# karfly/learnable-triangulation-pytorch

Hardware: NVIDIA H100
Metric: volumetric samples/sec (4-view 384x384, 64^3 grid) (higher is better)
Workload: dtype fp16x3 (split-fp16 operands, 3 wgmma products per term, fp32 accumulate)

## Files before the change

### include/lt_b200.h

```cpp
#ifndef LT_B200_H
#define LT_B200_H

#include <stddef.h>
#include <stdint.h>

#ifdef __cplusplus
extern "C" {
#endif

enum lt_status {
  LT_OK = 0,
  LT_ERR_INVALID = -1,
  LT_ERR_CUDA = -2,
  LT_ERR_UNSUPPORTED = -3
};

enum lt_format { LT_FMT_F32 = 0, LT_FMT_S32 = 1 };

enum lt_agg { LT_AGG_SUM = 0, LT_AGG_MAX = 1, LT_AGG_SOFTMAX = 2, LT_AGG_CONF = 3 };

enum lt_conv_impl {
  LT_CONV_SIMT = 0,
  LT_CONV_TC = 1,
  LT_CONV_TC1 = 2,
  LT_CONV_TC_FOLD = 3,
};

enum lt_residual { LT_RES_NONE = 0, LT_RES_BEFORE_RELU = 1, LT_RES_AFTER_RELU = 2 };

typedef struct lt_options {
  int tc_persist;
  int tc_splitk;
  int tc_bres;
  int tc_direct_epilogue;
  int fold_fast_issue;
  int fold_debug;
  int softargmax_stream;
  int unproject_v2;
  int unproject_cpl;
  int unproject_lb;
  int unproject_brick;
  int unproject_brick_order;
  int pair_nt, pair_stages;
  int pair_prof;
  int pair_direct_out;
  int pair_two_acc;
  int fold_pair;
  int fold_direct;
  int fold_fullw;
} lt_options;
void lt_default_options(lt_options* o);
int lt_get_options(lt_options* o);
int lt_set_options(const lt_options* o);

int lt_version(void);
const char* lt_last_error_string(void);

int lt_device_info(int* sm_count, int* cc_major, int* cc_minor);

int lt_coord_volume_fwd(const float* position, const float* center, const float* step, const float* rot,
                        float* out, int B, int n, int transfer_cmu, void* stream);

int lt_unproject_aggregate_fwd(const float* features, const float* proj, const float* coord, const float* conf,
                               void* out, int out_format, int B, int V, int C, int h, int w, long nvox,
                               int agg, void* stream);

int lt_unproject_partial_fwd(const float* features, const float* proj, const float* coord, const float* conf,
                             float* partial, int B, int V_local, int C, int h, int w, long nvox,
                             int agg, void* stream);
int lt_unproject_finalize_fwd(const float* partial, void* out, int out_format, int B, int C, long nvox,
                              int agg, void* stream);

int lt_unproject_push_fwd(const float* features, const float* proj, const float* coord, const float* conf,
                          float* const* peer_buffers , int n_peers, int src_rank,
                          int B, int V_local, int C, int h, int w, long nvox, int agg, void* stream);
int lt_unproject_reduce_finalize_fwd(const float* slots, int nslots, void* out, int out_format, int B, int C, long nvox,
                                     int agg, void* stream);

int lt_feature_scatter_fwd(const float* feats, float* const* peer_buffers, int n_peers, int view_rank, int B, int V_local,
                           int V, long row_elems, void* stream);

int lt_unproject_aggregate_bwd(const float* features, const float* proj, const float* coord, const float* conf,
// ... 17 lines not shown
int lt_softargmax3d_finish_fwd(const float* logits, long batch_stride, long voxel_stride, const float* coord, float* volumes_out,
                               float* keypoints_out, void* workspace, size_t workspace_bytes, int B, int J, long nvox, int G,
                               float multiplier, int softmax, void* stream);

typedef struct lt_conv_desc {
  int N, ID, IH, IW, Cin;
  int OD, OH, OW, Cout;
  int KD, KH, KW;
  int sd, sh, sw;
  int pd, ph, pw;
  int FD, FH, FW, FC;
  int osd, osh, osw;
  int ood, ooh, oow;
  int relu;
  int residual;
  int in_format, out_format;
  int ogd, ogh, ogw;
  int reserved0;
  void* workspace;
  size_t workspace_bytes;
} lt_conv_desc;

int lt_conv_nd_fwd(const lt_conv_desc* desc, const void* in, const void* weight, const float* scale,
                   const float* shift, const void* residual, void* out, int impl, void* stream);

size_t lt_conv_tc_weight_bytes(int taps, int Cin, int Cout);

typedef struct lt_conv_tc_launch_plan {
  int nt;
  int m_tiles, n_tiles;
  int chunks;
  int splits;
  int grid;
} lt_conv_tc_launch_plan;
int lt_conv_tc_plan(const lt_conv_desc* desc, int sm_count, int splitk, lt_conv_tc_launch_plan* plan);
int lt_conv_tc_pack_weights(const float* w_tap_ci_co, void* packed, int taps, int Cin, int Cout, void* stream);

int lt_absmax_fwd(const float* w, long n, unsigned int* out_bits, void* stream);
int lt_conv_gather_weights_fwd(const float* w, long base, long s_td, long s_th, long s_tw, long s_ci, long s_co, int KD, int KH, int KW,
                               int Cin, int CinP, int Cout, int CoutP, const unsigned int* absmax_bits, float* out, int out_ld,
                               int out_col0, void* stream);
int lt_fold_bn_fwd(const float* gamma, const float* beta, const float* mean, const float* var, const float* conv_bias, float eps,
                   int C, int CP, const unsigned int* absmax_bits, int accum_steps, float* scale, float* shift, void* stream);

int lt_v2v_tail_fwd(const void* x, const void* w1, const void* w2, const void* w3, const float* scale1, const float* shift1,
                    const float* scale2, const float* shift2, const float* scale3, const float* bias3, float* logits, long rows, int FC,
                    void* stream);
int lt_v2v_tail_stats_fwd(const void* x, const void* w1, const void* w2, const void* w3, const float* scale1, const float* shift1,
                          const float* scale2, const float* shift2, const float* scale3, const float* bias3, float* logits, int B,
                          long nvox, int FC, const float* coord, int J, float multiplier, int softmax, void* workspace,
                          size_t workspace_bytes, int* n_partials, void* stream);

size_t lt_conv_wgrad_workspace_bytes(const lt_conv_desc* desc);
typedef struct lt_conv_wgrad_launch_plan {
  int nwg;
  int ngroups;
  int m_tiles;
  int splits;
  int stages;
} lt_conv_wgrad_launch_plan;
int lt_conv_wgrad_plan(const lt_conv_desc* desc, int sm_count, lt_conv_wgrad_launch_plan* plan);
int lt_conv_wgrad_fwd(const lt_conv_desc* desc, const void* in, const void* grad_out, const unsigned int* grad_absmax_bits, int Cin,
                      int Cout, float* grad_w, void* workspace, size_t workspace_bytes, void* stream);

size_t lt_conv_fold_weight_bytes(int K, int Cout);
int lt_conv_fold_pack_weights(const float* w_tap_ci_co, void* packed, int K, int Cout, void* stream);
// ... 69 lines not shown
```

### learnable-triangulation-pytorch_b200/capi.py

```python
import ctypes
import os

import torch

from . import build as _build

_HERE = os.path.dirname(os.path.abspath(__file__))
LIB_PATH = os.path.join(_HERE, "liblt_b200.so")

FMT_F32, FMT_S32 = 0, 1
AGG = {"sum": 0, "max": 1, "softmax": 2, "conf": 3, "conf_norm": 3}
CONV_SIMT, CONV_TC, CONV_TC1, CONV_TC_FOLD = 0, 1, 2, 3
RES_NONE, RES_BEFORE_RELU, RES_AFTER_RELU = 0, 1, 2

c_int, c_long, c_float, c_void_p, c_size_t = ctypes.c_int, ctypes.c_long, ctypes.c_float, ctypes.c_void_p, ctypes.c_size_t


class ConvDesc(ctypes.Structure):
    _fields_ = [(n, c_int) for n in (
        "N", "ID", "IH", "IW", "Cin",
        "OD", "OH", "OW", "Cout",
        "KD", "KH", "KW",
        "sd", "sh", "sw",
        "pd", "ph", "pw",
        "FD", "FH", "FW", "FC",
        "osd", "osh", "osw",
        "ood", "ooh", "oow",
        "relu", "residual", "in_format", "out_format", "ogd", "ogh", "ogw", "reserved0")] + [("workspace", c_void_p), ("workspace_bytes", c_size_t)]


class ConvTcPlan(ctypes.Structure):
    _fields_ = [(n, c_int) for n in ("nt", "m_tiles", "n_tiles", "chunks", "splits", "grid")]


class ConvWgradPlan(ctypes.Structure):
    _fields_ = [(n, c_int) for n in ("nwg", "ngroups", "m_tiles", "splits", "stages")]


class Options(ctypes.Structure):
    _fields_ = [(n, c_int) for n in ("tc_persist", "tc_splitk", "tc_bres", "tc_direct_epilogue", "fold_fast_issue", "fold_debug",
                                     "softargmax_stream", "unproject_v2", "unproject_cpl", "unproject_lb", "unproject_brick", "unproject_brick_order", "pair_nt", "pair_stages", "pair_prof", "pair_direct_out", "pair_two_acc", "fold_pair", "fold_direct", "fold_fullw")]


OPTIONS_ENV_PREFIX = "LT_OPT_"

SIGNATURES = {
    "lt_default_options": (None, [ctypes.POINTER(Options)]),
    "lt_get_options": (c_int, [ctypes.POINTER(Options)]),
    "lt_set_options": (c_int, [ctypes.POINTER(Options)]),
    "lt_version": (c_int, []),
    "lt_last_error_string": (ctypes.c_char_p, []),
    "lt_device_info": (c_int, [ctypes.POINTER(c_int)] * 3),
    "lt_coord_volume_fwd": (c_int, [c_void_p] * 5 + [c_int, c_int, c_int, c_void_p]),
    "lt_unproject_aggregate_fwd": (c_int, [c_void_p] * 5 + [c_int] * 6 + [c_long, c_int, c_void_p]),
    "lt_unproject_partial_fwd": (c_int, [c_void_p] * 5 + [c_int] * 5 + [c_long, c_int, c_void_p]),
    "lt_unproject_finalize_fwd": (c_int, [c_void_p, c_void_p, c_int, c_int, c_int, c_long, c_int, c_void_p]),
    "lt_unproject_push_fwd": (c_int, [c_void_p] * 4 + [ctypes.POINTER(c_void_p), c_int, c_int] + [c_int] * 5 + [c_long, c_int, c_void_p]),
    "lt_unproject_reduce_finalize_fwd": (c_int, [c_void_p, c_int, c_void_p, c_int, c_int, c_int, c_long, c_int, c_void_p]),
    "lt_feature_scatter_fwd": (c_int, [c_void_p, ctypes.POINTER(c_void_p), c_int, c_int, c_int, c_int, c_int, c_long, c_void_p]),
    "lt_unproject_aggregate_bwd": (c_int, [c_void_p] * 7 + [c_int] * 5 + [c_long, c_int, c_void_p]),
    "lt_softargmax3d_bwd": (c_int, [c_void_p] * 6 + [c_int, c_int, c_long, c_float, c_int, c_void_p]),
    "lt_unproject_aggregate_bwd_geom_workspace_bytes": (c_size_t, [c_int, c_int, c_long]),
    "lt_unproject_aggregate_bwd_geom": (c_int, [c_void_p] * 10 + [c_size_t] + [c_int] * 5 + [c_long, c_int, c_void_p]),
    "lt_softargmax3d_coord_bwd": (c_int, [c_void_p] * 3 + [c_int, c_int, c_long, c_int, c_void_p]),
    "lt_test_unproject_aggregate_bwd_geom_host": (c_int, [c_void_p] * 9 + [c_int] * 5 + [c_long, c_int]),
    "lt_test_softargmax3d_coord_bwd_host": (c_int, [c_void_p] * 3 + [c_int, c_int, c_long]),
    "lt_test_unproject_aggregate_bwd_host": (c_int, [c_void_p] * 7 + [c_int] * 5 + [c_long, c_int]),
    "lt_test_softargmax3d_bwd_host": (c_int, [c_void_p] * 5 + [c_int, c_int, c_long, c_float, c_int]),
    "lt_softargmax3d_workspace_bytes": (c_size_t, [c_int, c_int, c_long]),
    "lt_softargmax3d_fwd": (c_int, [c_void_p, c_long, c_long, c_long, c_void_p, c_void_p, c_void_p, c_void_p, c_size_t,
                                    c_int, c_int, c_long, c_float, c_int, c_void_p]),
    "lt_conv_nd_fwd": (c_int, [ctypes.POINTER(ConvDesc)] + [c_void_p] * 6 + [c_int, c_void_p]),
    "lt_conv_tc_weight_bytes": (c_size_t, [c_int, c_int, c_int]),
    "lt_conv_tc_plan": (c_int, [ctypes.POINTER(ConvDesc), c_int, c_int, ctypes.POINTER(ConvTcPlan)]),
# ... 447 lines not shown
```

### learnable-triangulation-pytorch_b200/csrc/capi.cu

```cuda
#include "common.cuh"
#include <string.h>

namespace lt {

char* err_buf() {
  static thread_local char buf[512] = {0};
  return buf;
}

int fail(int code, const char* fmt, ...) {
  va_list ap;
  va_start(ap, fmt);
  vsnprintf(err_buf(), 512, fmt, ap);
  va_end(ap);
  return code;
}

static lt_options make_default_options() {
  lt_options o;
  o.tc_persist = 1; o.tc_splitk = 1; o.tc_bres = 1; o.tc_direct_epilogue = 0;
  o.fold_fast_issue = 1; o.fold_debug = 0;
  o.softargmax_stream = 1;
  o.unproject_v2 = 1; o.unproject_cpl = 4; o.unproject_lb = 0;
  o.unproject_brick = 0; o.unproject_brick_order = 2;
  o.pair_nt = 0; o.pair_stages = 0;
  o.pair_prof = 0;
  o.pair_direct_out = 1;
  o.pair_two_acc = 1;
  o.fold_pair = 1;
  o.fold_direct = 0;
  o.fold_fullw = 1;
  return o;
}
static lt_options g_options = make_default_options();
const lt_options& opts() { return g_options; }

int sm_count() {
  static thread_local int cached_dev = -1, cached = 0;
  int dev = 0;
  if (cudaGetDevice(&dev) != cudaSuccess) return 132;
  if (dev != cached_dev) {
    int n = 0;
    if (cudaDeviceGetAttribute(&n, cudaDevAttrMultiProcessorCount, dev) != cudaSuccess || n <= 0) n = 132;
    cached = n;
    cached_dev = dev;
  }
  return cached;
}

int conv_simt_fwd(const lt_conv_desc* d, const void* in, const void* weight, const float* scale, const float* shift,
                  const void* residual, void* out, void* stream);
int conv_tc_fwd_terms(const lt_conv_desc* d, const void* in, const void* weight, const float* scale, const float* shift,
                      const void* residual, void* out, int terms, void* stream);

int conv_fold_fwd(const lt_conv_desc* d, const void* in, const void* weight, const float* scale, const float* shift,
                  const void* residual, void* out, void* stream);

}

extern "C" int lt_version(void) { return 203; }

extern "C" void lt_default_options(lt_options* o) {
  if (o) *o = lt::make_default_options();
}
extern "C" int lt_get_options(lt_options* o) {
  if (!o) return lt::fail(LT_ERR_INVALID, "lt_get_options: null pointer");
  *o = lt::g_options;
  return LT_OK;
}
extern "C" int lt_set_options(const lt_options* o) {
  using namespace lt;
  LT_REQUIRE(o, "lt_set_options: null pointer");
  LT_REQUIRE(o->unproject_cpl == 4 || o->unproject_cpl == 8, "lt_set_options: unproject_cpl must be 4 or 8");
  LT_REQUIRE(o->tc_persist >= 0 && o->tc_persist <= 2, "lt_set_options: tc_persist must be 0, 1 or 2");
  g_options = *o;
  return LT_OK;
}

extern "C" const char* lt_last_error_string(void) { return lt::err_buf(); }

extern "C" int lt_device_info(int* sm_count, int* cc_major, int* cc_minor) {
  int dev = 0;
  if (cudaGetDevice(&dev) != cudaSuccess) return lt::fail(LT_ERR_CUDA, "no CUDA device");
  cudaDeviceProp prop;
  if (cudaGetDeviceProperties(&prop, dev) != cudaSuccess) return lt::fail(LT_ERR_CUDA, "cudaGetDeviceProperties failed");
  if (sm_count) *sm_count = prop.multiProcessorCount;
  if (cc_major) *cc_major = prop.major;
  if (cc_minor) *cc_minor = prop.minor;
  return LT_OK;
}

extern "C" int lt_conv_nd_fwd(const lt_conv_desc* d, const void* in, const void* weight, const float* scale,
                              const float* shift, const void* residual, void* out, int impl, void* stream) {
  using namespace lt;
  LT_REQUIRE(d && in && weight && scale && shift && out, "conv_nd: null pointer");
  LT_REQUIRE(d->N > 0 && d->ID > 0 && d->IH > 0 && d->IW > 0 && d->Cin > 0, "conv_nd: bad input dims");
  LT_REQUIRE(d->OD > 0 && d->OH > 0 && d->OW > 0 && d->Cout > 0, "conv_nd: bad output dims");
  LT_REQUIRE(d->KD > 0 && d->KH > 0 && d->KW > 0 && d->sd > 0 && d->sh > 0 && d->sw > 0, "conv_nd: bad filter/stride");
  LT_REQUIRE(d->osd > 0 && d->osh > 0 && d->osw > 0, "conv_nd: bad output scale");
  const int gd = d->ogd > 1 ? d->ogd : 1, gh = d->ogh > 1 ? d->ogh : 1, gw = d->ogw > 1 ? d->ogw : 1;
  LT_REQUIRE((d->OD - 1) * d->osd + d->ood < d->FD && (d->OH - 1) * d->osh + d->ooh < d->FH && (d->OW - 1) * d->osw + d->oow < d->FW &&
                 d->ood + gd - 1 < d->FD && d->ooh + gh - 1 < d->FH && d->oow + gw - 1 < d->FW && d->ood >= 0 && d->ooh >= 0 &&
                 d->oow >= 0,
             "conv_nd: output mapping exceeds the output tensor");
  LT_REQUIRE(gd * gh * gw == 1 || impl == LT_CONV_TC || impl == LT_CONV_TC1,
             "conv_nd: grouped output (ogd/ogh/ogw) is only implemented by the tensor-core kernels");
  LT_REQUIRE(d->residual == LT_RES_NONE || residual, "conv_nd: residual requested but pointer is null");
// ... 8 lines not shown
```

### learnable-triangulation-pytorch_b200/csrc/conv_tc.cu

```cuda
#include "tc_common.cuh"
#include "conv_tc_params.cuh"
#include <stdlib.h>
#include <string.h>

namespace lt {

constexpr int kTcThreads = 384;

struct TcUnit {
  int m, n0, z, q_begin, nchunks;
};
__device__ __forceinline__ TcUnit tc_unit(const TcParams& p, int u, int m_tiles, int nchunks_all) {
  TcUnit w;
  const int n = u % p.n_tiles;
  u /= p.n_tiles;
  w.m = u % m_tiles;
  w.z = u / m_tiles;
  w.n0 = n * p.Nt;
  w.q_begin = (int)(((long)w.z * nchunks_all) / p.splits);
  w.nchunks = (int)(((long)(w.z + 1) * nchunks_all) / p.splits) - w.q_begin;
  return w;
}
__device__ __forceinline__ void tc_tile_origin(const TcParams& p, int t, int& ow0, int& oh0, int& od0, int& nb0) {
  ow0 = (t % p.tw) * p.bw; t /= p.tw;
  oh0 = (t % p.th) * p.bh; t /= p.th;
  od0 = (t % p.td) * p.bd;
  nb0 = (t / p.td) * p.bn;
}

constexpr int kSlabBytes = 128 * 128;
__host__ __device__ constexpr int tc_epi_bytes(int nt, int splits) { return (nt >= 32 && splits == 1) ? nt / 32 * kSlabBytes : 0; }

__device__ __forceinline__ void epi_slab(const TcParams& p, int co, int& g, int& c) {
  g = p.n_maps > 1 ? co / p.oc : 0;
  const int ch = co - g * p.oc;
  c = p.out_format == LT_FMT_F32 ? ch : 2 * ch;
}

__device__ __forceinline__ uint32_t sw128(int row, int b) {
  return (uint32_t)(row * 128 + ((((b >> 4) ^ row) & 7) << 4) + (b & 15));
}

template <int NT>
__global__ void __launch_bounds__(kTcThreads, 1) conv_tc_kernel(const __grid_constant__ CUtensorMap tmA,
                                                                const __grid_constant__ CUtensorMap tmB,
                                                                const __grid_constant__ TcEpiMaps tmE, const TcParams p) {
  extern __shared__ uint8_t smem_raw[];
  uint8_t* smem = reinterpret_cast<uint8_t*>((reinterpret_cast<uintptr_t>(smem_raw) + 1023) & ~(uintptr_t)1023);
  constexpr int kStage = kATileBytes + NT * 128;
  const int epi_bytes = tc_epi_bytes(NT, p.splits);
  const bool staged = epi_bytes > 0;
  uint8_t* ebuf = smem + (size_t)p.stages * kStage;
  uint64_t* full = reinterpret_cast<uint64_t*>(ebuf + epi_bytes);
  uint64_t* empty = full + p.stages;
  uint64_t* efull = empty + p.stages;
  uint64_t* edone = efull + 1;

  const int wg = __shfl_sync(0xffffffffu, (int)(threadIdx.x >> 7), 0);
  const int lane = threadIdx.x & 31;
  const int m_tiles = p.tw * p.th * p.td * p.tn;
  const int units = m_tiles * p.n_tiles * p.splits;
  const int nchunks_all = p.KD * p.KH * p.KW * p.CB;

  if (threadIdx.x == 0) {
    for (int s = 0; s < p.stages; ++s) { mbar_init(&full[s], 1); mbar_init(&empty[s], 2); }
    mbar_init(efull, 1);
    mbar_init(edone, 256);
    fence_barrier_init();
    prefetch_tmap(&tmA);
    prefetch_tmap(&tmB);
  }
  __syncthreads();

  if (wg == 0) {
    regs_release_producer();
    if (staged && threadIdx.x == 32) {
      uint32_t eph = 0;
      for (int u = blockIdx.x; u < units; u += gridDim.x) {
        const TcUnit w = tc_unit(p, u, m_tiles, nchunks_all);
        int ow0, oh0, od0, nb0;
        tc_tile_origin(p, w.m, ow0, oh0, od0, nb0);
        bulk_wait_read0();
        if (p.residual != LT_RES_NONE) {
          mbar_expect_tx(efull, (uint32_t)epi_bytes);
          for (int sl = 0; sl < NT / 32; ++sl) {
            int g, c;
            epi_slab(p, w.n0 + 32 * sl, g, c);
            tma_load_5d(ebuf + sl * kSlabBytes, &tmE.res[g], efull, c, ow0, oh0, od0, nb0);
          }
        } else {
          mbar_arrive_local(efull);
        }
        mbar_wait(edone, eph);
        eph ^= 1u;
        for (int sl = 0; sl < NT / 32; ++sl) {
          int g, c;
          epi_slab(p, w.n0 + 32 * sl, g, c);
          tma_store_5d(&tmE.out[g], ebuf + sl * kSlabBytes, c, ow0, oh0, od0, nb0);
        }
        bulk_commit();
      }
      bulk_wait0();
    }
    if (threadIdx.x < 32) {
      int s = 0;
      uint32_t ph = 0;
      for (int u = blockIdx.x; u < units; u += gridDim.x) {
        const TcUnit w = tc_unit(p, u, m_tiles, nchunks_all);
        int ow0, oh0, od0, nb0;
        tc_tile_origin(p, w.m, ow0, oh0, od0, nb0);
        int tap = w.q_begin / p.CB, cb = w.q_begin - tap * p.CB;
        int kw = tap % p.KW, kh = (tap / p.KW) % p.KH, kd = tap / (p.KW * p.KH);
        const int ax = ow0 * p.sw - p.pw, ay = oh0 * p.sh - p.ph, az = od0 * p.sd - p.pd, bn0 = w.n0 * p.b_nmul;
        for (int q = 0, qa = w.q_begin; q < w.nchunks; ++q, ++qa) {
          mbar_wait(&empty[s], ph ^ 1u);
          uint8_t* a_dst = smem + (size_t)s * kStage;
          if (elect_one()) {
            mbar_expect_tx(&full[s], (uint32_t)kStage);
            tma_load_5d(a_dst, &tmA, &full[s], cb * 64, ax + kw, ay + kh, az + kd, nb0);
            tma_load_2d(a_dst + kATileBytes, &tmB, &full[s], qa * p.b_step0, qa * p.b_step1 + bn0);
          }
          __syncwarp();
          if (++cb == p.CB) { cb = 0; if (++kw == p.KW) { kw = 0; if (++kh == p.KH) { kh = 0; ++kd; } } }
          if (++s == p.stages) { s = 0; ph ^= 1u; }
        }
      }
    }
    return;
  }

  regs_claim_consumer();
  const int g = wg - 1;
  float d1[NT / 2], d2[NT / 2];
#pragma unroll
  for (int i = 0; i < NT / 2; ++i) { d1[i] = 0.f; d2[i] = 0.f; }
  const int r0 = g * 64 + ((threadIdx.x >> 5) & 3) * 16 + (lane >> 2);
  const int c2 = 2 * (lane & 3);
  const uint32_t ring0 = smem_u32(smem);
  int s = 0;
  uint32_t ph = 0, eph = 0;
  for (int u = blockIdx.x; u < units; u += gridDim.x) {
    const TcUnit w = tc_unit(p, u, m_tiles, nchunks_all);
    int prev = -1;
    for (int q = 0; q < w.nchunks; ++q) {
      mbar_wait(&full[s], ph);
      const uint32_t a_addr = ring0 + (uint32_t)(s * kStage) + (uint32_t)(g * 64 * 128);
      const uint32_t b_addr = ring0 + (uint32_t)(s * kStage) + kATileBytes;
      const uint64_t ad = make_sw128_desc(a_addr), bd = make_sw128_desc(b_addr);
      const uint32_t acc = (q == 0) ? 0u : 1u;
      wg_fence();
      if (p.terms == 3) {
        wgmma_f16<NT>(d1, ad, bd, acc);
        wgmma_f16<NT>(d1, ad + 2, bd + 2, 1u);
        wgmma_f16<NT>(d2, ad, bd + 4, acc);
        wgmma_f16<NT>(d2, ad + 2, bd + 6, 1u);
        wgmma_f16<NT>(d2, ad + 4, bd, 1u);
        wgmma_f16<NT>(d2, ad + 6, bd + 2, 1u);
      } else if (p.terms == 1) {
        wgmma_f16<NT>(d1, ad, bd, acc);
        wgmma_f16<NT>(d1, ad + 2, bd + 2, 1u);
      } else {
        wgmma_f16<NT>(d1, ad, bd, acc);
        wgmma_f16<NT>(d1, ad + 2, bd + 2, 1u);
        wgmma_f16<NT>(d1, ad + 4, bd + 4, 1u);
        wgmma_f16<NT>(d1, ad + 6, bd + 6, 1u);
      }
      wg_commit();
      wg_wait<1>();
      if (prev >= 0 && (threadIdx.x & 127) == 0) mbar_arrive_local(&empty[prev]);
      prev = s;
      if (++s == p.stages) { s = 0; ph ^= 1u; }
    }
    wg_wait<0>();
    if (prev >= 0 && (threadIdx.x & 127) == 0) mbar_arrive_local(&empty[prev]);
    wg_fence_regs(d1);
    wg_fence_regs(d2);

    if (p.splits > 1) {
#pragma unroll
      for (int h = 0; h < 2; ++h) {
        float* wrow = p.ws + (((size_t)w.z * m_tiles + w.m) * 128 + r0 + 8 * h) * p.ws_ld + w.n0;
#pragma unroll
        for (int i = 0; i < NT / 8; ++i) {
          const int k = 4 * i + 2 * h;
          const float v0 = (p.terms == 3) ? fmaf(d2[k], kLoInv, d1[k]) : d1[k];
          const float v1 = (p.terms == 3) ? fmaf(d2[k + 1], kLoInv, d1[k + 1]) : d1[k + 1];
          *reinterpret_cast<float2*>(wrow + 8 * i + c2) = make_float2(v0, v1);
        }
      }
      continue;
    }
    if constexpr (NT >= 32) {
      mbar_wait(efull, eph);
      eph ^= 1u;
      const uint32_t e0 = smem_u32(ebuf);
      auto fc_ok = [&](int co) {
        int ch;
        long pix;
        epilogue_target(p, co, 0, ch, pix);
        return ch < p.FC;
      };
      float2 sc = make_float2(0.f, 0.f), sh = sc;
      if (fc_ok(w.n0 + c2)) {
        sc = __ldg(reinterpret_cast<const float2*>(p.scale + w.n0 + c2));
        sh = __ldg(reinterpret_cast<const float2*>(p.shift + w.n0 + c2));
      }
#pragma unroll
      for (int i = 0; i < NT / 8; ++i) {
        const int co = w.n0 + 8 * i + c2;
        const bool ok = fc_ok(co);
        float2 sc_next = sc, sh_next = sh;
        if (i + 1 < NT / 8 && fc_ok(co + 8)) {
          sc_next = __ldg(reinterpret_cast<const float2*>(p.scale + co + 8));
          sh_next = __ldg(reinterpret_cast<const float2*>(p.shift + co + 8));
        }
        const uint32_t slab = e0 + (uint32_t)((i >> 2) * kSlabBytes);
        const int cc = 8 * (i & 3) + c2;
#pragma unroll
        for (int h = 0; h < 2 && ok; ++h) {
          const int row = r0 + 8 * h;
          const int k = 4 * i + 2 * h;
          float v0 = (p.terms == 3) ? fmaf(d2[k], kLoInv, d1[k]) : d1[k];
          float v1 = (p.terms == 3) ? fmaf(d2[k + 1], kLoInv, d1[k + 1]) : d1[k + 1];
          v0 = fmaf(v0, sc.x, sh.x);
          v1 = fmaf(v1, sc.y, sh.y);
          if (p.out_format == LT_FMT_F32) {
            const uint32_t a = slab + sw128(row, 4 * cc);
            float2 r = make_float2(0.f, 0.f);
            if (p.residual != LT_RES_NONE) r = lds_f2(a);
            if (p.residual == LT_RES_BEFORE_RELU) { v0 += r.x; v1 += r.y; }
            if (p.relu) { v0 = fmaxf(v0, 0.f); v1 = fmaxf(v1, 0.f); }
            if (p.residual == LT_RES_AFTER_RELU) { v0 += r.x; v1 += r.y; }
            sts_f2(a, make_float2(v0, v1));
          } else {
            const uint32_t ahi = slab + sw128(row, 2 * cc), alo = slab + sw128(row, 64 + 2 * cc);
            float2 r = make_float2(0.f, 0.f);
            if (p.residual != LT_RES_NONE) {
              const uint32_t rh = lds32(ahi), rl = lds32(alo);
              const float2 a = __half22float2(*reinterpret_cast<const __half2*>(&rh));
              const float2 b = __half22float2(*reinterpret_cast<const __half2*>(&rl));
              r = make_float2(fmaf(b.x, kLoInv, a.x), fmaf(b.y, kLoInv, a.y));
            }
            if (p.residual == LT_RES_BEFORE_RELU) { v0 += r.x; v1 += r.y; }
            if (p.relu) { v0 = fmaxf(v0, 0.f); v1 = fmaxf(v1, 0.f); }
            if (p.residual == LT_RES_AFTER_RELU) { v0 += r.x; v1 += r.y; }
            uint32_t hi2, lo2;
            split_s32x2(v0, v1, hi2, lo2);
            sts32(ahi, hi2);
            sts32(alo, lo2);
          }
        }
        sc = sc_next;
        sh = sh_next;
      }
      fence_proxy_async();
      mbar_arrive_local(edone);
    } else {
      int ow0, oh0, od0, nb0;
      tc_tile_origin(p, w.m, ow0, oh0, od0, nb0);
#pragma unroll
      for (int h = 0; h < 2; ++h) {
        int r_ = r0 + 8 * h;
        const int dw = r_ % p.bw; r_ /= p.bw;
        const int dh = r_ % p.bh; r_ /= p.bh;
        const int dd = r_ % p.bd; r_ /= p.bd;
        const int ow = ow0 + dw, oh = oh0 + dh, od = od0 + dd, nb = nb0 + r_;
        if (!(ow < p.OW && oh < p.OH && od < p.OD && nb < p.N)) continue;
        const long opix = (((long)nb * p.FD + (od * p.osd + p.ood)) * p.FH + (oh * p.osh + p.ooh)) * p.FW + (ow * p.osw + p.oow);
        conv_epilogue_row<NT>(p, d1, d2, h, opix, w.n0, c2);
      }
    }
  }
}

typedef CUresult (*EncodeTiledFn)(CUtensorMap*, CUtensorMapDataType, cuuint32_t, void*, const cuuint64_t*, const cuuint64_t*,
                                  const cuuint32_t*, const cuuint32_t*, CUtensorMapInterleave, CUtensorMapSwizzle,
                                  CUtensorMapL2promotion, CUtensorMapFloatOOBfill);

static EncodeTiledFn encode_fn() {
  static EncodeTiledFn fn = nullptr;
  if (!fn) {
    void* ptr = nullptr;
    cudaDriverEntryPointQueryResult qres;
    if (cudaGetDriverEntryPoint("cuTensorMapEncodeTiled", &ptr, cudaEnableDefault, &qres) == cudaSuccess &&
        qres == cudaDriverEntryPointSuccess)
      fn = reinterpret_cast<EncodeTiledFn>(ptr);
  }
  return fn;
}
// ... 150 lines not shown
  }
  const long units = tiles * best;
  *splits_out = best;
  *grid_out = (int)(units < sm ? units : sm);
}

static int group_extent(int n, int F, int off, int ph, int os) {
  const int e = (F - off - ph + os - 1) / os;
  return e < n ? e : n;
}

static int make_epi_maps(const TcParams& p, TcEpiMaps* m) {
  const int f32 = p.out_format == LT_FMT_F32;
  const uint64_t rowb = (uint64_t)p.FC * 4;
  const uint64_t str[4] = {rowb * p.osw, rowb * p.FW * p.osh, rowb * p.FW * p.FH * p.osd, rowb * p.FW * p.FH * p.FD};
  const uint32_t bx[5] = {f32 ? 32u : 64u, (uint32_t)p.bw, (uint32_t)p.bh, (uint32_t)p.bd, (uint32_t)p.bn};
  for (int g = 0; g < p.n_maps; ++g) {
    const int ga = g / (p.gh * p.gw), gb = (g / p.gw) % p.gh, gc = g % p.gw;
    const int ew = group_extent(p.OW, p.FW, p.oow, gc, p.osw), eh = group_extent(p.OH, p.FH, p.ooh, gb, p.osh),
              ed = group_extent(p.OD, p.FD, p.ood, ga, p.osd);
    LT_REQUIRE(ew > 0 && eh > 0 && ed > 0, "conv_tc: output group %d lies outside the %dx%dx%d output tensor", g, p.FD, p.FH, p.FW);
    const uint64_t dims[5] = {(uint64_t)(f32 ? p.FC : 2 * p.FC), (uint64_t)ew, (uint64_t)eh, (uint64_t)ed, (uint64_t)p.N};
    const long pix0 = ((long)(p.ood + ga) * p.FH + p.ooh + gb) * p.FW + p.oow + gc;
    int rc = make_map(&m->out[g], static_cast<const uint8_t*>(p.out) + pix0 * rowb, 5, dims, str, bx, nullptr, 1, f32);
    if (rc) return rc;
    if (p.residual == LT_RES_NONE) continue;
    rc = make_map(&m->res[g], static_cast<const uint8_t*>(p.res) + pix0 * rowb, 5, dims, str, bx, nullptr, 1, f32);
    if (rc) return rc;
  }
  return LT_OK;
}

constexpr int kTcSmemBudget = 224 * 1024;

static int launch_tc(const CUtensorMap& tmA, const CUtensorMap& tmB, TcParams& p, int n_tiles, cudaStream_t st, void* ws = nullptr,
                     size_t ws_bytes = 0) {
  const long m_tiles = (long)p.tw * p.th * p.td * p.tn;
  int splits, grid;
  tc_plan(m_tiles, n_tiles, p.Nt, p.KD * p.KH * p.KW * p.CB, p.terms, p.n_maps, ws ? opts().tc_splitk : 0, ws_bytes, sm_count(),
          &splits, &grid);
  p.splits = splits;
  const double steps = 2.0 * p.KD * p.KH * p.KW * p.CB;
  p.ws_gain = (float)(accum_gain(steps / splits) / accum_gain(steps));
  p.ws = reinterpret_cast<float*>(ws);
  p.ws_ld = n_tiles * p.Nt;
  p.n_tiles = n_tiles;
  const int stage_bytes = kATileBytes + p.Nt * 128;
  const int epi_bytes = tc_epi_bytes(p.Nt, splits);
  int stages = (kTcSmemBudget - epi_bytes) / stage_bytes;
  if (stages > 8) stages = 8;
  p.stages = stages;
  const size_t smem = (size_t)stages * stage_bytes + epi_bytes + (2 * stages + 2) * 8 + 1024;
  TcEpiMaps tmE{};
  int rc;
  if (epi_bytes) {
    rc = make_epi_maps(p, &tmE);
    if (rc) return rc;
  }
  switch (p.Nt) {
    case 128: rc = launch_nt<128>(tmA, tmB, tmE, p, dim3(grid), smem, st); break;
    case 64: rc = launch_nt<64>(tmA, tmB, tmE, p, dim3(grid), smem, st); break;
    case 32: rc = launch_nt<32>(tmA, tmB, tmE, p, dim3(grid), smem, st); break;
    case 16: rc = launch_nt<16>(tmA, tmB, tmE, p, dim3(grid), smem, st); break;
    default: return fail(LT_ERR_INVALID, "conv_tc: unsupported N tile %d", p.Nt);
  }
  if (rc) return rc;
  if (splits > 1) {
    const long total = m_tiles * 128 * (p.ws_ld / 4);
    long blocks = (total + 255) / 256;
    if (blocks > 4L * sm_count()) blocks = 4L * sm_count();
    splitk_reduce_kernel<<<(unsigned)blocks, 256, 0, st>>>(p, m_tiles, p.ws_ld);
    cudaError_t e = cudaGetLastError();
    if (e != cudaSuccess) return fail(LT_ERR_CUDA, "splitk_reduce_kernel: %s", cudaGetErrorString(e));
  }
  return LT_OK;
}

void fill_params(const lt_conv_desc* d, TcParams& p, int CB, int CoutP, int Nt, int terms, const float* scale, const float* shift,
                        const void* residual, void* out) {
  p.OW = d->OW; p.OH = d->OH; p.OD = d->OD; p.N = d->N;
  int box[4];
  pick_box(d->OW, d->OH, d->OD, d->N, box);
  p.bw = box[0]; p.bh = box[1]; p.bd = box[2]; p.bn = box[3];
  p.tw = ceil_div(d->OW, p.bw); p.th = ceil_div(d->OH, p.bh); p.td = ceil_div(d->OD, p.bd); p.tn = ceil_div(d->N, p.bn);
  p.KW = d->KW; p.KH = d->KH; p.KD = d->KD; p.pw = d->pw; p.ph = d->ph; p.pd = d->pd;
  p.sw = d->sw; p.sh = d->sh; p.sd = d->sd;
  p.CB = CB; p.b_step0 = 0; p.b_step1 = CoutP; p.b_nmul = 1; p.Nt = Nt; p.terms = terms;
  p.FC = d->FC; p.FD = d->FD; p.FH = d->FH; p.FW = d->FW;
  p.osd = d->osd; p.osh = d->osh; p.osw = d->osw; p.ood = d->ood; p.ooh = d->ooh; p.oow = d->oow;
  p.relu = d->relu; p.residual = d->residual; p.out_format = d->out_format;
  p.scale = scale; p.shift = shift; p.res = residual; p.out = out;
  p.splits = 1; p.ws = nullptr; p.ws_ld = 0; p.ws_gain = 1.0f; p.stages = 0; p.n_tiles = 1;
  p.n_maps = out_groups(d);
  p.oc = p.n_maps > 1 ? d->Cout / p.n_maps : CoutP;
  p.gh = d->ogh > 1 ? d->ogh : 1; p.gw = d->ogw > 1 ? d->ogw : 1;
}

int make_in_map(CUtensorMap* tmA, const lt_conv_desc* d, int bw, int bh, int bd, int bn, const void* in) {
  const uint64_t rowb = (uint64_t)d->Cin * 2 * 2;
  const uint64_t dims[5] = {(uint64_t)d->Cin * 2, (uint64_t)d->IW, (uint64_t)d->IH, (uint64_t)d->ID, (uint64_t)d->N};
  const uint64_t str[4] = {rowb, rowb * d->IW, rowb * d->IW * d->IH, rowb * d->IW * d->IH * d->ID};
  const uint32_t es[5] = {1, (uint32_t)d->sw, (uint32_t)d->sh, (uint32_t)d->sd, 1};
  uint32_t bx[5] = {64, (uint32_t)bw, (uint32_t)bh, (uint32_t)bd, (uint32_t)bn};
  for (int i = 1; i <= 3; ++i) bx[i] = (bx[i] - 1) * es[i] + 1;
  LT_REQUIRE(bx[1] <= 256 && bx[2] <= 256 && bx[3] <= 256, "conv_tc: strided box exceeds 256");
  return make_map(tmA, in, 5, dims, str, bx, es, 1);
}

static bool groups_ok(const lt_conv_desc* d, int CoutP) {
  const int G = out_groups(d);
  return d->Cout % G == 0 && (d->Cout / G) % 32 == 0 && d->Cout / G == d->FC && CoutP == d->Cout && G <= kMaxOutMaps;
}

int conv_tc_fwd_terms(const lt_conv_desc* d, const void* in, const void* weight, const float* scale, const float* shift,
                      const void* residual, void* out, int terms, void* stream) {
  LT_REQUIRE(d->in_format == LT_FMT_S32, "conv_tc: input must be split-fp16");
  LT_REQUIRE(d->Cin % 32 == 0, "conv_tc: Cin=%d must be a multiple of 32", d->Cin);
  LT_REQUIRE(d->FC % 4 == 0 && (d->out_format == LT_FMT_F32 || d->FC % 32 == 0), "conv_tc: bad output channel stride %d", d->FC);
  LT_REQUIRE((reinterpret_cast<uintptr_t>(out) | reinterpret_cast<uintptr_t>(residual)) % 16 == 0,
             "conv_tc: out and residual must be 16-byte aligned (TMA global addresses)");
  const int CoutP = (d->Cout + 15) & ~15;
  const int CB = d->Cin / 32;
  const int taps = d->KD * d->KH * d->KW;
  const int Nt = pick_nt(CoutP);
  TcParams p;
// ... 23 lines not shown
    const int n = (int)(r % CoutP); r /= CoutP;
    const int cb = (int)(r % CB);
    const int tap = (int)(r / CB);
    const float v = (n < Cout) ? w[((long)tap * Cin + cb * 32 + j) * Cout + n] : 0.0f;
    sh_t hi, lo;
    split_s32(v, hi, lo);
    sh_t* rowp = out + ((((long)tap * CB + cb) * CoutP + n) << 6);
    rowp[j] = hi;
    rowp[32 + j] = lo;
  }
}

__global__ void ones_zeros_kernel(float* ones, float* zeros, int n) {
  const int i = blockIdx.x * blockDim.x + threadIdx.x;
  if (i < n) { ones[i] = 1.0f; zeros[i] = 0.0f; }
}

}

using namespace lt;

extern "C" int lt_conv_tc_plan(const lt_conv_desc* d, int sm_count, int splitk, lt_conv_tc_launch_plan* plan) {
  LT_REQUIRE(d && plan && sm_count > 0, "conv_tc_plan: bad arguments");
  LT_REQUIRE(d->Cin % 32 == 0 && d->Cout > 0, "conv_tc_plan: Cin=%d must be a multiple of 32", d->Cin);
  const int CoutP = (d->Cout + 15) & ~15;
  int box[4];
  pick_box(d->OW, d->OH, d->OD, d->N, box);
  plan->nt = pick_nt(CoutP);
  plan->m_tiles = ceil_div(d->OW, box[0]) * ceil_div(d->OH, box[1]) * ceil_div(d->OD, box[2]) * ceil_div(d->N, box[3]);
  plan->n_tiles = CoutP / plan->nt;
  plan->chunks = d->KD * d->KH * d->KW * (d->Cin / 32);
  tc_plan(plan->m_tiles, plan->n_tiles, plan->nt, plan->chunks, 3, out_groups(d), d->workspace ? splitk : 0, d->workspace_bytes,
          sm_count, &plan->splits, &plan->grid);
  return LT_OK;
}

extern "C" size_t lt_conv_tc_weight_bytes(int taps, int Cin, int Cout) {
  const int CoutP = (Cout + 15) & ~15;
  return (size_t)taps * (Cin / 32) * CoutP * 128;
}

extern "C" int lt_conv_tc_pack_weights(const float* w, void* packed, int taps, int Cin, int Cout, void* stream) {
  LT_REQUIRE(w && packed, "conv_tc_pack_weights: null pointer");
  LT_REQUIRE(Cin % 32 == 0 && taps > 0 && Cout > 0, "conv_tc_pack_weights: bad sizes");
  const int CoutP = (Cout + 15) & ~15;
  const long total = (long)taps * (Cin / 32) * CoutP * 32;
  long blocks = (total + 255) / 256;
  if (blocks > 65535) blocks = 65535;
  pack_weights_kernel<<<(unsigned)blocks, 256, 0, (cudaStream_t)stream>>>(w, reinterpret_cast<sh_t*>(packed), taps, Cin, Cout, CoutP);
  LT_CHECK_LAUNCH("pack_weights_kernel");
  return LT_OK;
}

extern "C" int lt_tc_gemm_selftest(const void* a, const void* b, float* d, int M, int N, int K, int variant, void* stream) {
  LT_REQUIRE(a && b && d, "tc_gemm_selftest: null pointer");
  LT_REQUIRE(M > 0 && N % 16 == 0 && N >= 16 && K % 64 == 0, "tc_gemm_selftest: need N %% 16 == 0, K %% 64 == 0");
  (void)variant;
  const int Nt = pick_nt(N);
  float* ones = d + (size_t)M * N;
  float* zeros = ones + N;
  ones_zeros_kernel<<<ceil_div(N, 256), 256, 0, (cudaStream_t)stream>>>(ones, zeros, N);
  TcParams p;
  p.OW = M; p.OH = 1; p.OD = 1; p.N = 1;
  p.bw = 128; p.bh = 1; p.bd = 1; p.bn = 1;
  p.tw = ceil_div(M, 128); p.th = 1; p.td = 1; p.tn = 1;
  p.KW = p.KH = p.KD = 1; p.pw = p.ph = p.pd = 0; p.sw = p.sh = p.sd = 1;
  p.CB = K / 64; p.b_step0 = 64; p.b_step1 = 0; p.b_nmul = 1; p.Nt = Nt; p.terms = 0;
  p.FC = N; p.FD = 1; p.FH = 1; p.FW = M; p.osd = p.osh = p.osw = 1; p.ood = p.ooh = p.oow = 0;
  p.relu = 0; p.residual = LT_RES_NONE; p.out_format = LT_FMT_F32;
  p.scale = ones; p.shift = zeros; p.res = nullptr; p.out = d;
  p.n_maps = 1; p.oc = N; p.gh = p.gw = 1;
  p.splits = 1; p.ws = nullptr; p.ws_ld = 0; p.ws_gain = 1.0f; p.n_tiles = 1;
  CUtensorMap tmA, tmB;
  {
    const uint64_t dims[5] = {(uint64_t)K, (uint64_t)M, 1, 1, 1};
    const uint64_t str[4] = {(uint64_t)K * 2, (uint64_t)K * 2 * M, (uint64_t)K * 2 * M, (uint64_t)K * 2 * M};
    const uint32_t bx[5] = {64, 128, 1, 1, 1};
    int rc = make_map(&tmA, a, 5, dims, str, bx, nullptr, 1);
    if (rc) return rc;
  }
  {
    const uint64_t dims[2] = {(uint64_t)K, (uint64_t)N};
    const uint64_t str[1] = {(uint64_t)K * 2};
    const uint32_t bx[2] = {64, (uint32_t)Nt};
    int rc = make_map(&tmB, b, 2, dims, str, bx, nullptr, 1);
    if (rc) return rc;
  }
  return launch_tc(tmA, tmB, p, N / Nt, (cudaStream_t)stream);
}
```

### learnable-triangulation-pytorch_b200/csrc/conv_tc_params.cuh

```cuda
#pragma once
#include "tc_common.cuh"

namespace lt {

struct TcParams {
  int OW, OH, OD, N;
  int bw, bh, bd, bn;
  int tw, th, td, tn;
  int KW, KH, KD, pw, ph, pd;
  int sw, sh, sd;
  int CB;
  int b_step0, b_step1;
  int b_nmul;
  int Nt, stages, terms;
  int FC, FD, FH, FW, osd, osh, osw, ood, ooh, oow, relu, residual, out_format;
  const float* scale;
  const float* shift;
  const void* res;
  void* out;
  int splits, ws_ld;
  float* ws;
  float ws_gain;
  int n_tiles;
  int oc, n_maps;
  int gh, gw;
};

constexpr int kMaxOutMaps = 8;

struct TcEpiMaps {
  CUtensorMap out[kMaxOutMaps];
  CUtensorMap res[kMaxOutMaps];
};

constexpr int kATileBytes = 128 * 128;

__device__ __forceinline__ void epilogue_target(const TcParams& p, int co, long opix, int& ch, long& pix) {
  ch = co;
  pix = opix;
  if (p.n_maps > 1) {
    const int mi = ch / p.oc;
    ch -= mi * p.oc;
    pix += ((long)(mi / (p.gh * p.gw)) * p.FH + (mi / p.gw) % p.gh) * p.FW + mi % p.gw;
  }
}

template <int NT>
__device__ __forceinline__ float2 epilogue_residual(const TcParams& p, int ch, long pix) {
  if (p.residual == LT_RES_NONE || ch >= p.FC) return make_float2(0.f, 0.f);
  if (p.out_format == LT_FMT_F32) return *reinterpret_cast<const float2*>(reinterpret_cast<const float*>(p.res) + pix * p.FC + ch);
  const sh_t* rp = reinterpret_cast<const sh_t*>(p.res) + pix * 2 * p.FC + s32_off(ch);
  const float2 a = __half22float2(*reinterpret_cast<const __half2*>(rp));
  const float2 b = __half22float2(*reinterpret_cast<const __half2*>(rp + 32));
  return make_float2(fmaf(b.x, kLoInv, a.x), fmaf(b.y, kLoInv, a.y));
}

template <int NT>
__device__ __forceinline__ void conv_epilogue_row(const TcParams& p, const float (&d1)[NT / 2], const float (&d2)[NT / 2], int h,
// ... 46 lines not shown
```

Baseline: 209.8.

## Keep A tiles stationary in shared memory across N tiles and double-buffer epilogue

```diff
diff --git a/include/lt_b200.h b/include/lt_b200.h
--- a/include/lt_b200.h
+++ b/include/lt_b200.h
@@ -48,6 +48,7 @@
   int fold_pair;
   int fold_direct;
   int fold_fullw;
+  int tc_stationary;
 } lt_options;
 void lt_default_options(lt_options* o);
 int lt_get_options(lt_options* o);
@@ -131,6 +132,9 @@
   int chunks;
   int splits;
   int grid;
+  int stationary;
+  int stages;
+  int epi_bufs;
 } lt_conv_tc_launch_plan;
 int lt_conv_tc_plan(const lt_conv_desc* desc, int sm_count, int splitk, lt_conv_tc_launch_plan* plan);
 int lt_conv_tc_pack_weights(const float* w_tap_ci_co, void* packed, int taps, int Cin, int Cout, void* stream);
diff --git a/learnable-triangulation-pytorch_b200/capi.py b/learnable-triangulation-pytorch_b200/capi.py
--- a/learnable-triangulation-pytorch_b200/capi.py
+++ b/learnable-triangulation-pytorch_b200/capi.py
@@ -30,7 +30,7 @@
 
 
 class ConvTcPlan(ctypes.Structure):
-    _fields_ = [(n, c_int) for n in ("nt", "m_tiles", "n_tiles", "chunks", "splits", "grid")]
+    _fields_ = [(n, c_int) for n in ("nt", "m_tiles", "n_tiles", "chunks", "splits", "grid", "stationary", "stages", "epi_bufs")]
 
 
 class ConvWgradPlan(ctypes.Structure):
@@ -39,7 +39,8 @@
 
 class Options(ctypes.Structure):
     _fields_ = [(n, c_int) for n in ("tc_persist", "tc_splitk", "tc_bres", "tc_direct_epilogue", "fold_fast_issue", "fold_debug",
-                                     "softargmax_stream", "unproject_v2", "unproject_cpl", "unproject_lb", "unproject_brick", "unproject_brick_order", "pair_nt", "pair_stages", "pair_prof", "pair_direct_out", "pair_two_acc", "fold_pair", "fold_direct", "fold_fullw")]
+                                     "softargmax_stream", "unproject_v2", "unproject_cpl", "unproject_lb", "unproject_brick", "unproject_brick_order", "pair_nt", "pair_stages", "pair_prof", "pair_direct_out", "pair_two_acc", "fold_pair", "fold_direct", "fold_fullw",
+                                     "tc_stationary")]
 
 
 OPTIONS_ENV_PREFIX = "LT_OPT_"
diff --git a/learnable-triangulation-pytorch_b200/csrc/capi.cu b/learnable-triangulation-pytorch_b200/csrc/capi.cu
--- a/learnable-triangulation-pytorch_b200/csrc/capi.cu
+++ b/learnable-triangulation-pytorch_b200/csrc/capi.cu
@@ -30,6 +30,7 @@
   o.fold_pair = 1;
   o.fold_direct = 0;
   o.fold_fullw = 1;
+  o.tc_stationary = 1;
   return o;
 }
 static lt_options g_options = make_default_options();
@@ -73,6 +74,7 @@
   LT_REQUIRE(o, "lt_set_options: null pointer");
   LT_REQUIRE(o->unproject_cpl == 4 || o->unproject_cpl == 8, "lt_set_options: unproject_cpl must be 4 or 8");
   LT_REQUIRE(o->tc_persist >= 0 && o->tc_persist <= 2, "lt_set_options: tc_persist must be 0, 1 or 2");
+  LT_REQUIRE(o->tc_stationary >= 0 && o->tc_stationary <= 2, "lt_set_options: tc_stationary must be 0, 1 or 2");
   g_options = *o;
   return LT_OK;
 }
diff --git a/learnable-triangulation-pytorch_b200/csrc/conv_tc.cu b/learnable-triangulation-pytorch_b200/csrc/conv_tc.cu
--- a/learnable-triangulation-pytorch_b200/csrc/conv_tc.cu
+++ b/learnable-triangulation-pytorch_b200/csrc/conv_tc.cu
@@ -47,25 +47,35 @@
                                                                 const __grid_constant__ TcEpiMaps tmE, const TcParams p) {
   extern __shared__ uint8_t smem_raw[];
   uint8_t* smem = reinterpret_cast<uint8_t*>((reinterpret_cast<uintptr_t>(smem_raw) + 1023) & ~(uintptr_t)1023);
-  constexpr int kStage = kATileBytes + NT * 128;
-  const int epi_bytes = tc_epi_bytes(NT, p.splits);
-  const bool staged = epi_bytes > 0;
-  uint8_t* ebuf = smem + (size_t)p.stages * kStage;
-  uint64_t* full = reinterpret_cast<uint64_t*>(ebuf + epi_bytes);
-  uint64_t* empty = full + p.stages;
-  uint64_t* efull = empty + p.stages;
-  uint64_t* edone = efull + 1;
-
-  const int wg = __shfl_sync(0xffffffffu, (int)(threadIdx.x >> 7), 0);
-  const int lane = threadIdx.x & 31;
+  constexpr int kBBytes = NT * 128;
   const int m_tiles = p.tw * p.th * p.td * p.tn;
   const int units = m_tiles * p.n_tiles * p.splits;
   const int nchunks_all = p.KD * p.KH * p.KW * p.CB;
+  const bool stationary = p.stationary != 0;
+  const int a_slots = stationary ? nchunks_all : 0;
+  const int stage_bytes = stationary ? kBBytes : kATileBytes + kBBytes;
+  const int epi_bytes = tc_epi_bytes(NT, p.splits);
+  const bool staged = epi_bytes > 0;
+  const int nbuf = p.epi_bufs;
+  uint8_t* ring = smem + (size_t)a_slots * kATileBytes;
+  uint8_t* ebuf = ring + (size_t)p.stages * stage_bytes;
+  uint64_t* full = reinterpret_cast<uint64_t*>(ebuf + (size_t)nbuf * epi_bytes);
+  uint64_t* empty = full + p.stages;
+  uint64_t* afull = empty + p.stages;
+  uint64_t* aempty = afull + a_slots;
+  uint64_t* efull = aempty + a_slots;
+  uint64_t* edone = efull + nbuf;
+
+  const int wg = __shfl_sync(0xffffffffu, (int)(threadIdx.x >> 7), 0);
+  const int lane = threadIdx.x & 31;
+  const int u_begin = stationary ? (int)(((long)blockIdx.x * units) / gridDim.x) : (int)blockIdx.x;
+  const int u_end = stationary ? (int)(((long)(blockIdx.x + 1) * units) / gridDim.x) : units;
+  const int u_step = stationary ? 1 : (int)gridDim.x;
 
   if (threadIdx.x == 0) {
     for (int s = 0; s < p.stages; ++s) { mbar_init(&full[s], 1); mbar_init(&empty[s], 2); }
-    mbar_init(efull, 1);
-    mbar_init(edone, 256);
+    for (int q = 0; q < a_slots; ++q) { mbar_init(&afull[q], 1); mbar_init(&aempty[q], 2); }
+    for (int b = 0; b < nbuf; ++b) { mbar_init(&efull[b], 1); mbar_init(&edone[b], 256); }
     fence_barrier_init();
     prefetch_tmap(&tmA);
     prefetch_tmap(&tmB);
@@ -75,55 +85,80 @@
   if (wg == 0) {
     regs_release_producer();
     if (staged && threadIdx.x == 32) {
-      uint32_t eph = 0;
-      for (int u = blockIdx.x; u < units; u += gridDim.x) {
+      auto fill = [&](int u, int b) {
         const TcUnit w = tc_unit(p, u, m_tiles, nchunks_all);
         int ow0, oh0, od0, nb0;
         tc_tile_origin(p, w.m, ow0, oh0, od0, nb0);
-        bulk_wait_read0();
         if (p.residual != LT_RES_NONE) {
-          mbar_expect_tx(efull, (uint32_t)epi_bytes);
+          mbar_expect_tx(&efull[b], (uint32_t)epi_bytes);
           for (int sl = 0; sl < NT / 32; ++sl) {
             int g, c;
             epi_slab(p, w.n0 + 32 * sl, g, c);
-            tma_load_5d(ebuf + sl * kSlabBytes, &tmE.res[g], efull, c, ow0, oh0, od0, nb0);
+            tma_load_5d(ebuf + (size_t)b * epi_bytes + sl * kSlabBytes, &tmE.res[g], &efull[b], c, ow0, oh0, od0, nb0);
           }
         } else {
-          mbar_arrive_local(efull);
+          mbar_arrive_local(&efull[b]);
         }
-        mbar_wait(edone, eph);
-        eph ^= 1u;
+      };
+      if (u_begin < u_end) fill(u_begin, 0);
+      int k = 0;
+      for (int u = u_begin; u < u_end; u += u_step, ++k) {
+        const int b = k % nbuf;
+        const bool more = u + u_step < u_end;
+        if (nbuf == 2 && more) {
+          bulk_wait_read0();
+          fill(u + u_step, b ^ 1);
+        }
+        const TcUnit w = tc_unit(p, u, m_tiles, nchunks_all);
+        int ow0, oh0, od0, nb0;
+        tc_tile_origin(p, w.m, ow0, oh0, od0, nb0);
+        mbar_wait(&edone[b], (uint32_t)(k / nbuf) & 1u);
         for (int sl = 0; sl < NT / 32; ++sl) {
           int g, c;
           epi_slab(p, w.n0 + 32 * sl, g, c);
-          tma_store_5d(&tmE.out[g], ebuf + sl * kSlabBytes, c, ow0, oh0, od0, nb0);
+          tma_store_5d(&tmE.out[g], ebuf + (size_t)b * epi_bytes + sl * kSlabBytes, c, ow0, oh0, od0, nb0);
         }
         bulk_commit();
+        if (nbuf == 1 && more) {
+          bulk_wait_read0();
+          fill(u + u_step, 0);
+        }
       }
       bulk_wait0();
     }
     if (threadIdx.x < 32) {
       int s = 0;
-      uint32_t ph = 0;
-      for (int u = blockIdx.x; u < units; u += gridDim.x) {
+      uint32_t ph = 0, aph = 0;
+      for (int u = u_begin; u < u_end; u += u_step) {
         const TcUnit w = tc_unit(p, u, m_tiles, nchunks_all);
+        const bool load_a = !stationary || u == u_begin || w.n0 == 0;
         int ow0, oh0, od0, nb0;
         tc_tile_origin(p, w.m, ow0, oh0, od0, nb0);
         int tap = w.q_begin / p.CB, cb = w.q_begin - tap * p.CB;
         int kw = tap % p.KW, kh = (tap / p.KW) % p.KH, kd = tap / (p.KW * p.KH);
         const int ax = ow0 * p.sw - p.pw, ay = oh0 * p.sh - p.ph, az = od0 * p.sd - p.pd, bn0 = w.n0 * p.b_nmul;
         for (int q = 0, qa = w.q_begin; q < w.nchunks; ++q, ++qa) {
+          if (stationary && load_a) mbar_wait(&aempty[q], aph ^ 1u);
           mbar_wait(&empty[s], ph ^ 1u);
-          uint8_t* a_dst = smem + (size_t)s * kStage;
+          uint8_t* b_dst = ring + (size_t)s * stage_bytes + (stationary ? 0 : kATileBytes);
           if (elect_one()) {
-            mbar_expect_tx(&full[s], (uint32_t)kStage);
-            tma_load_5d(a_dst, &tmA, &full[s], cb * 64, ax + kw, ay + kh, az + kd, nb0);
-            tma_load_2d(a_dst + kATileBytes, &tmB, &full[s], qa * p.b_step0, qa * p.b_step1 + bn0);
+            if (!stationary) {
+              mbar_expect_tx(&full[s], (uint32_t)(kATileBytes + kBBytes));
+              tma_load_5d(ring + (size_t)s * stage_bytes, &tmA, &full[s], cb * 64, ax + kw, ay + kh, az + kd, nb0);
+            } else {
+              if (load_a) {
+                mbar_expect_tx(&afull[q], (uint32_t)kATileBytes);
+                tma_load_5d(smem + (size_t)q * kATileBytes, &tmA, &afull[q], cb * 64, ax + kw, ay + kh, az + kd, nb0);
+              }
+              mbar_expect_tx(&full[s], (uint32_t)kBBytes);
+            }
+            tma_load_2d(b_dst, &tmB, &full[s], qa * p.b_step0, qa * p.b_step1 + bn0);
           }
           __syncwarp();
           if (++cb == p.CB) { cb = 0; if (++kw == p.KW) { kw = 0; if (++kh == p.KH) { kh = 0; ++kd; } } }
           if (++s == p.stages) { s = 0; ph ^= 1u; }
         }
+        if (stationary && load_a) aph ^= 1u;
       }
     }
     return;
@@ -136,16 +171,18 @@
   for (int i = 0; i < NT / 2; ++i) { d1[i] = 0.f; d2[i] = 0.f; }
   const int r0 = g * 64 + ((threadIdx.x >> 5) & 3) * 16 + (lane >> 2);
   const int c2 = 2 * (lane & 3);
-  const uint32_t ring0 = smem_u32(smem);
-  int s = 0;
-  uint32_t ph = 0, eph = 0;
-  for (int u = blockIdx.x; u < units; u += gridDim.x) {
+  const uint32_t a_rows = (uint32_t)(g * 64 * 128), slots0 = smem_u32(smem), ring0 = smem_u32(ring);
+  int s = 0, k = 0;
+  uint32_t ph = 0, aph = 0;
+  for (int u = u_begin; u < u_end; u += u_step, ++k) {
     const TcUnit w = tc_unit(p, u, m_tiles, nchunks_all);
+    const bool release_a = stationary && (u + 1 == u_end || w.n0 + NT == p.n_tiles * NT);
     int prev = -1;
     for (int q = 0; q < w.nchunks; ++q) {
+      if (stationary) mbar_wait(&afull[q], aph);
       mbar_wait(&full[s], ph);
-      const uint32_t a_addr = ring0 + (uint32_t)(s * kStage) + (uint32_t)(g * 64 * 128);
-      const uint32_t b_addr = ring0 + (uint32_t)(s * kStage) + kATileBytes;
+      const uint32_t a_addr = (stationary ? slots0 + (uint32_t)(q * kATileBytes) : ring0 + (uint32_t)(s * stage_bytes)) + a_rows;
+      const uint32_t b_addr = ring0 + (uint32_t)(s * stage_bytes) + (stationary ? 0u : (uint32_t)kATileBytes);
       const uint64_t ad = make_sw128_desc(a_addr), bd = make_sw128_desc(b_addr);
       const uint32_t acc = (q == 0) ? 0u : 1u;
       wg_fence();
@@ -167,12 +204,19 @@
       }
       wg_commit();
       wg_wait<1>();
-      if (prev >= 0 && (threadIdx.x & 127) == 0) mbar_arrive_local(&empty[prev]);
+      if (prev >= 0 && (threadIdx.x & 127) == 0) {
+        mbar_arrive_local(&empty[prev]);
+        if (release_a) mbar_arrive_local(&aempty[q - 1]);
+      }
       prev = s;
       if (++s == p.stages) { s = 0; ph ^= 1u; }
     }
     wg_wait<0>();
-    if (prev >= 0 && (threadIdx.x & 127) == 0) mbar_arrive_local(&empty[prev]);
+    if (prev >= 0 && (threadIdx.x & 127) == 0) {
+      mbar_arrive_local(&empty[prev]);
+      if (release_a) mbar_arrive_local(&aempty[w.nchunks - 1]);
+    }
+    if (release_a) aph ^= 1u;
     wg_fence_regs(d1);
     wg_fence_regs(d2);
 
@@ -191,9 +235,9 @@
       continue;
     }
     if constexpr (NT >= 32) {
-      mbar_wait(efull, eph);
-      eph ^= 1u;
-      const uint32_t e0 = smem_u32(ebuf);
+      const int b = k % nbuf;
+      mbar_wait(&efull[b], (uint32_t)(k / nbuf) & 1u);
+      const uint32_t e0 = smem_u32(ebuf + (size_t)b * epi_bytes);
       auto fc_ok = [&](int co) {
         int ch;
         long pix;
@@ -254,7 +298,7 @@
         sh = sh_next;
       }
       fence_proxy_async();
-      mbar_arrive_local(edone);
+      mbar_arrive_local(&edone[b]);
     } else {
       int ow0, oh0, od0, nb0;
       tc_tile_origin(p, w.m, ow0, oh0, od0, nb0);
@@ -471,25 +515,52 @@
 }
 
 constexpr int kTcSmemBudget = 224 * 1024;
+constexpr int kTcStationaryABytes = 128 * 1024;
+
+struct TcSchedule {
+  int stationary, stages, epi_bufs;
+  size_t smem;
+};
+static TcSchedule tc_schedule(int nt, int chunks, int n_tiles, int splits, int mode) {
+  const int epi = tc_epi_bytes(nt, splits), b_bytes = nt * 128, a_bytes = chunks * kATileBytes;
+  TcSchedule sc{0, 0, 1, 0};
+  if (mode != 0 && epi > 0 && a_bytes <= kTcStationaryABytes && (mode == 2 || n_tiles >= 2) &&
+      kTcSmemBudget - a_bytes - epi >= 2 * b_bytes) {
+    const int rest = kTcSmemBudget - a_bytes;
+    const int bufs = rest - 2 * epi >= 2 * b_bytes ? 2 : 1;
+    const int stages = (rest - bufs * epi) / b_bytes;
+    if (mode == 2 || (bufs == 2 && stages >= 4)) {
+      sc.stationary = 1;
+      sc.epi_bufs = bufs;
+      sc.stages = stages;
+    }
+  }
+  if (!sc.stationary) sc.stages = (kTcSmemBudget - epi) / (kATileBytes + b_bytes);
+  if (sc.stages > 8) sc.stages = 8;
+  const int a_slots = sc.stationary ? chunks : 0;
+  sc.smem = (size_t)sc.stages * (b_bytes + (sc.stationary ? 0 : kATileBytes)) + (size_t)a_slots * kATileBytes +
+            (size_t)sc.epi_bufs * epi + (2 * sc.stages + 2 * a_slots + 2 * sc.epi_bufs) * 8 + 1024;
+  return sc;
+}
 
 static int launch_tc(const CUtensorMap& tmA, const CUtensorMap& tmB, TcParams& p, int n_tiles, cudaStream_t st, void* ws = nullptr,
                      size_t ws_bytes = 0) {
   const long m_tiles = (long)p.tw * p.th * p.td * p.tn;
+  const int chunks = p.KD * p.KH * p.KW * p.CB;
   int splits, grid;
-  tc_plan(m_tiles, n_tiles, p.Nt, p.KD * p.KH * p.KW * p.CB, p.terms, p.n_maps, ws ? opts().tc_splitk : 0, ws_bytes, sm_count(),
-          &splits, &grid);
+  tc_plan(m_tiles, n_tiles, p.Nt, chunks, p.terms, p.n_maps, ws ? opts().tc_splitk : 0, ws_bytes, sm_count(), &splits, &grid);
   p.splits = splits;
   const double steps = 2.0 * p.KD * p.KH * p.KW * p.CB;
   p.ws_gain = (float)(accum_gain(steps / splits) / accum_gain(steps));
   p.ws = reinterpret_cast<float*>(ws);
   p.ws_ld = n_tiles * p.Nt;
   p.n_tiles = n_tiles;
-  const int stage_bytes = kATileBytes + p.Nt * 128;
   const int epi_bytes = tc_epi_bytes(p.Nt, splits);
-  int stages = (kTcSmemBudget - epi_bytes) / stage_bytes;
-  if (stages > 8) stages = 8;
-  p.stages = stages;
-  const size_t smem = (size_t)stages * stage_bytes + epi_bytes + (2 * stages + 2) * 8 + 1024;
+  const TcSchedule sc = tc_schedule(p.Nt, chunks, n_tiles, splits, opts().tc_stationary);
+  p.stationary = sc.stationary;
+  p.stages = sc.stages;
+  p.epi_bufs = sc.epi_bufs;
+  const size_t smem = sc.smem;
   TcEpiMaps tmE{};
   int rc;
   if (epi_bytes) {
@@ -530,6 +601,7 @@
   p.relu = d->relu; p.residual = d->residual; p.out_format = d->out_format;
   p.scale = scale; p.shift = shift; p.res = residual; p.out = out;
   p.splits = 1; p.ws = nullptr; p.ws_ld = 0; p.ws_gain = 1.0f; p.stages = 0; p.n_tiles = 1;
+  p.stationary = 0; p.epi_bufs = 1;
   p.n_maps = out_groups(d);
   p.oc = p.n_maps > 1 ? d->Cout / p.n_maps : CoutP;
   p.gh = d->ogh > 1 ? d->ogh : 1; p.gw = d->ogw > 1 ? d->ogw : 1;
@@ -619,6 +691,10 @@
   plan->chunks = d->KD * d->KH * d->KW * (d->Cin / 32);
   tc_plan(plan->m_tiles, plan->n_tiles, plan->nt, plan->chunks, 3, out_groups(d), d->workspace ? splitk : 0, d->workspace_bytes,
           sm_count, &plan->splits, &plan->grid);
+  const TcSchedule sc = tc_schedule(plan->nt, plan->chunks, plan->n_tiles, plan->splits, opts().tc_stationary);
+  plan->stationary = sc.stationary;
+  plan->stages = sc.stages;
+  plan->epi_bufs = sc.epi_bufs;
   return LT_OK;
 }
 
@@ -658,6 +734,7 @@
   p.scale = ones; p.shift = zeros; p.res = nullptr; p.out = d;
   p.n_maps = 1; p.oc = N; p.gh = p.gw = 1;
   p.splits = 1; p.ws = nullptr; p.ws_ld = 0; p.ws_gain = 1.0f; p.n_tiles = 1;
+  p.stationary = 0; p.epi_bufs = 1;
   CUtensorMap tmA, tmB;
   {
     const uint64_t dims[5] = {(uint64_t)K, (uint64_t)M, 1, 1, 1};
diff --git a/learnable-triangulation-pytorch_b200/csrc/conv_tc_params.cuh b/learnable-triangulation-pytorch_b200/csrc/conv_tc_params.cuh
--- a/learnable-triangulation-pytorch_b200/csrc/conv_tc_params.cuh
+++ b/learnable-triangulation-pytorch_b200/csrc/conv_tc_params.cuh
@@ -24,6 +24,7 @@
   int n_tiles;
   int oc, n_maps;
   int gh, gw;
+  int stationary, epi_bufs;
 };
 
 constexpr int kMaxOutMaps = 8;
```

Measured after the change: 214.8, median of 6. 2.4% higher.
